# cartographer-project/cartographer

Hardware: AMD Instinct MI355X
Metric: candidate poses scored/sec (higher is better)
Workload: dtype u8/int32; 1 GPU; C2: 2D FastCorrelativeScanMatcher MatchFullSubmap (branch and bound): 1000-point scan vs 1 400x400 submap(s) per GPU, depth 7, full-angle search, m...; submaps_per_gpu=1, rotations=2373, found=1

## Files before the change

cartographer_amd/csrc/cmx_common.h:

```cpp
#ifndef CMX_COMMON_H_
#define CMX_COMMON_H_

#include <hip/hip_runtime.h>

#include <cstdarg>
#include <cstdint>
#include <cstdio>
#include <cstring>
#include <functional>
#include <mutex>
#include <string>
#include <vector>

#include "../../include/cartographer_mi355x.h"

namespace cmx {

void SetLastError(const char* fmt, ...);
const char* LastError();

struct HipError {
  cmx_status status;
};

// ... 30 lines not shown
    SetLastError("exception: %s", e.what());
    return CMX_DEVICE_ERROR;
  }
}

#define CMX_DEBUG_OPTIONS(X)                                                                      \
  X(rt2d_legacy)                 \
  X(rt2d_tile)                                        \
  X(rt2d_groups)                                   \
  X(rt2d_target)                                    \
  X(rt2d_lds_kb)                                         \
  X(rt2d_no_image_cache)             \
  X(rt2d_parts)                                 \
  X(rt2d_host_par)         \
  X(rt2d_tables_serial)    \
  X(rt2d_first_part)       \
  X(rt2d_image_kernels)    \
  X(rt2d_no_lane)          \
  X(rt2d_parts_pool)       \
  X(rt2d_grid_share)       \
  X(rt2d_unfused)            \
  X(rt2d_no_bounds)        \
  X(rt2d_bounds)           \
  X(rt2d_bounds_fused)     \
  X(rt2d_bounds_level)     \
  X(rt2d_bounds_verify)    \
  X(rt2d_tsdf_batch_legacy)  \
  X(rt2d_tsdf_batch_bulk)  \
  X(rt2d_tsdf_verify)      \
  X(timeline)                  \
  X(trace)                       \
  X(host_trace)                          \
  X(launch_serial)         \
  X(sync)                      \
  X(no_copy_kernels)             \
  X(timing)                \
  X(no_direct_results)     \
  X(frontier_capacity)     \
  X(comm_virtual_ranks)    \
  X(comm_force_rccl)       \
  X(fast2d_unfused)                    \
  X(fast2d_store_scans)                   \
  X(fast2d_fused_threads)                            \
  X(fast2d_fanout)         \
  X(fast2d_group)          \
  X(fast2d_group_verify)   \
  X(fast2d_levels_per_stage)                                    \
  X(fast2d_wave_levels)                        \
  X(fast2d_xcd_affinity)                          \
  X(fast2d_queue)          \
  X(fast2d_queue_blocks)                \
  X(fast2d_queue_capacity)              \
  X(fast2d_queue_lost)       \
  X(filters_generic)       \
  X(fast3d_byte_loads)                             \
  X(fast3d_affinity)                              \
  X(fast3d_no_families)                             \
  X(fast3d_no_oct)                                         \
  X(fast3d_batch)                                                 \
  X(fast3d_chunk_cells)    \
  X(rt3d_legacy)                  \
  X(rt3d_no_tiles)                      \
  X(rt3d_verify)                  \
  X(rt3d_no_rotblocks)              \
  X(rt3d_rotblock_permille)  \
  X(rt3d_crosscheck)           \
  X(rt3d_expand_all)       \
  X(rt3d_unstaged)                                     \
  X(rt3d_no_boxes)                            \
  X(rt3d_report)                                             \
  X(rt3d_segments)                         \
  X(rt3d_group_rotations)                                  \
  X(rt3d_group_tile_kb)                                   \
  X(rt3d_group_float)                          \
  X(rt3d_cand_threads)                                   \
  X(rt3d_cand_rotations)                                    \
  X(rt3d_cand_tile_kb)
struct DebugOptions {
#define CMX_DEBUG_FIELD(name) int name = 0;
  CMX_DEBUG_OPTIONS(CMX_DEBUG_FIELD)
#undef CMX_DEBUG_FIELD
};
const DebugOptions& Debug();
bool DebugSet(const char* name, int value);

void UseDevice(int device);

void ParallelFor(int n, int serial_below, const std::function<void(int)>& fn);

class LaunchTurn {
 public:
  LaunchTurn();
  ~LaunchTurn();
  LaunchTurn(const LaunchTurn&) = delete;
  LaunchTurn& operator=(const LaunchTurn&) = delete;
 private:
  bool held_;
};

class HostLane {
 public:
  HostLane();
  ~HostLane();
  HostLane(const HostLane&) = delete;
  HostLane& operator=(const HostLane&) = delete;
  void Run(std::function<void()> fn);
// ... 157 lines not shown
```

cartographer_amd/csrc/fast_2d.hip:

```cpp
#include <algorithm>
#include <chrono>
#include <cstring>
#include <memory>
#include <type_traits>
#include <utility>

#include "fast_2d_device.h"
#include "fast_2d_internal.h"

namespace cmx {
namespace {

constexpr int kSeedsPerProblem = 64;

constexpr int kMaxStages = kMaxDepth + 2;

constexpr int kCountStride = 32;
constexpr int kQueues = 2048;
struct alignas(8) QueueCtl {
  int head;
  int reserved;
  int pad[30];
};
struct Counters {
  int frontier[kMaxStages][kSubLists * kCountStride];
  int leaves[kSubLists * kCountStride];
  int frontier_overflow;
  int leaf_overflow;
  unsigned wave_gathers;
  int blocks_done;
  int pad[28];
  unsigned gathers_shard[16 * kCountStride];
  unsigned queue_stats[16 * kCountStride];
  QueueCtl queue[kQueues];
};

struct CountersSummary {
  int leaves[kSubLists];
  int frontier_total[kMaxStages];
  int frontier_overflow;
  int leaf_overflow;
  unsigned wave_gathers;
  int pad;
  unsigned queue_stats[8];
};

struct NodeList {
  Node2D* nodes;
  int* counts;
  int sub_capacity;
};

__device__ __forceinline__ int ListReserve(const NodeList& list, int sub, int m) {
  return atomicAdd(&list.counts[sub * kCountStride], m);
}
__device__ __forceinline__ bool ListStore(const NodeList& list, int sub, int slot,
                                          const Node2D& nd) {
  if (slot >= list.sub_capacity) return false;
  list.nodes[static_cast<size_t>(sub) * list.sub_capacity + slot] = nd;
  return true;
}
__device__ __forceinline__ int ListMaxCount(const NodeList& list) {
  const int lane = threadIdx.x & 63;
  return WaveMax(min(list.counts[lane * kCountStride], list.sub_capacity));
}

__device__ __forceinline__ int NodeProblem(const Node2D& nd) { return nd.problem & 0xffffff; }
__device__ __forceinline__ int NodeLevel(const Node2D& nd) { return nd.problem >> 24; }

__device__ __forceinline__ Node2D CoarseNode(const Fast2DProblem& P, int problem, int s,
                                             int local) {
  const int2 dims = P.coarse_dims[s];
  const int4 bd = P.bounds[s];
  const int step = 1 << (P.depth - 1);
  const int ix = local / dims.y, iy = local - ix * dims.y;
  const int c = s * P.coarse_stride + local;
  Node2D nd;
  nd.problem = problem | ((P.depth - 1) << 24);
  nd.scan = s;
  nd.dx = bd.x + ix * step;
  nd.dy = bd.z + iy * step;
  nd.score = P.coarse_score[c];
  nd.coarse_index = c;
  nd.path = 0;
  nd.coarse_score = nd.score;
  return nd;
}

struct SeedScratch {
  int hist[1024];
  int wave_total[4];
  int threshold_bin;
  int found_scan;
  int total;
};

__device__ __forceinline__ bool PickSeed(const Fast2DProblem& P, int n, int want,
                                         SeedScratch* sh, int* scan_out) {
  const int tid = threadIdx.x, lane = tid & 63, T = blockDim.x;
  for (int i = tid; i < 1024; i += T) sh->hist[i] = 0;
  if (tid == 0) { sh->found_scan = -1; sh->total = 0; }
  __syncthreads();
  const int S = P.num_scans;
  const long long range = 255ll * n + 1;
  const auto* scan_best = AsGlobal(P.scan_best);
  const auto* coarse_dims = AsGlobal(P.coarse_dims);
  const bool grouped = P.group > 1;
  const auto best_of = [&](int s) -> int {
    if (grouped) {
      const int first = s - s % kFusedGroup;
      if (s != first + (S - first >= kFusedGroup ? 1 : 0)) return -1;
    }
    return scan_best[s].x;
  };
  constexpr int kOwn = 16;
  int own[kOwn];
#pragma unroll
  for (int k = 0; k < kOwn; ++k) {
    const int s = tid + k * T;
    own[k] = s < S ? best_of(s) : -1;
  }
  int total = 0;
#pragma unroll
  for (int k = 0; k < kOwn; ++k)
    if (own[k] >= 0) atomicAdd(&sh->hist[static_cast<int>(own[k] * 1024ll / range)], 1);
  for (int s = tid + kOwn * T; s < S; s += T) {
    const int b = best_of(s);
    if (b >= 0) atomicAdd(&sh->hist[static_cast<int>(b * 1024ll / range)], 1);
  }
  if (want == 0) {
    for (int s = tid; s < S; s += T) total += coarse_dims[s].x * coarse_dims[s].y;
    total = WaveSum(total);
    if (lane == 0 && total) atomicAdd(&sh->total, total);
  }
  __syncthreads();
  if (tid < 64) {
    int mine = 0;
#pragma unroll
    for (int k = 0; k < 16; ++k) mine += sh->hist[1023 - 16 * lane - k];
// ... 168 lines not shown
  };
  if (quads_by_buffer) {
    if (cached) walk(std::true_type{}, std::true_type{});
    else walk(std::false_type{}, std::true_type{});
  } else {
    if (cached) walk(std::true_type{}, std::false_type{});
    else walk(std::false_type{}, std::false_type{});
  }
  s00 = WaveSum(s00); s01 = WaveSum(s01); s10 = WaveSum(s10); s11 = WaveSum(s11);
  const int wave = threadIdx.x >> 6;
  if ((threadIdx.x & 63) == 0) {
    sh->partial[wave][0] = s00; sh->partial[wave][1] = s01;
    sh->partial[wave][2] = s10; sh->partial[wave][3] = s11;
  }
  __syncthreads();
  if (threadIdx.x < 64) {
    const int k = threadIdx.x & 3;
    const bool valid = ((k >> 1) == 0 || vx) && ((k & 1) == 0 || vy);
    const int total = sh->partial[0][k] + sh->partial[1][k] + sh->partial[2][k] + sh->partial[3][k];
    const float mine = valid ? ToScoreCtx(ctx, total) : -1.f;
    int rank = 0, nvalid = 0;
#pragma unroll
    for (int j = 0; j < 4; ++j) {
      const float other = __shfl(mine, j, 64);
      if (other >= 0.f) ++nvalid;
      if (j != k && other >= 0.f && (other > mine || (other == mine && j < k))) ++rank;
    }
    if (threadIdx.x < 4) {
      sh->child_score[k] = mine;
      sh->rank[k] = rank;
      if (k == 0) sh->nvalid = nvalid;
    }
  }
  __syncthreads();
}

__device__ __forceinline__ Node2D MakeChild(const Node2D& nd, int k, int child_level,
                                            const ChildScratch& sh) {
  Node2D child = nd;
  child.problem = NodeProblem(nd) | (child_level << 24);
  child.dx = nd.dx + (k >> 1) * (1 << child_level);
  child.dy = nd.dy + (k & 1) * (1 << child_level);
  child.score = sh.child_score[k];
  child.path = nd.path | (static_cast<unsigned>(sh.rank[k]) << (2 * child_level));
  return child;
}

__device__ __forceinline__ void RecordLeaf(const Node2D& leaf, const NodeList& leaves,
                                           Counters* __restrict__ counters) {
  const int sub = blockIdx.x & (kSubLists - 1);
  if (!ListStore(leaves, sub, ListReserve(leaves, sub, 1), leaf)) counters->leaf_overflow = 1;
}

__global__ void __launch_bounds__(256, 4)
DiveKernel(const Fast2DProblem* __restrict__ problems, ProblemState* __restrict__ states, int n,
           NodeList leaves, Counters* __restrict__ counters) {
  const int problem = blockIdx.y;
  const Fast2DProblem& P = problems[problem];
  ProblemState& st = states[problem];
  if (st.error) return;
  __shared__ BlockContext ctx;
  __shared__ ChildScratch sh;
  __shared__ Node2D cur;
  __shared__ SeedScratch seed_scratch;
  const int per_seed = P.group > 1 ? kFusedGroup : 1;
  if (static_cast<int>(blockIdx.x) >= kSeedsPerProblem * per_seed) return;
  int seed_scan;
  const bool have_seed = PickSeed(P, n, blockIdx.x / per_seed, &seed_scratch, &seed_scan);
  if (blockIdx.x == 0 && threadIdx.x == 0) st.coarse_total = seed_scratch.total;
  if (!have_seed) return;
  if (per_seed > 1) {
    seed_scan = seed_scan - seed_scan % kFusedGroup + static_cast<int>(blockIdx.x) % per_seed;
    if (seed_scan >= P.num_scans) return;
  }
  const Node2D seed = CoarseNode(P, problem, seed_scan, P.scan_best[seed_scan].y);
  if (threadIdx.x == 0) cur = seed;
  LoadContext(P, n, seed.scan, &ctx);
  const int depth = NodeLevel(seed) + 1;
  unsigned long long scored = 0;
  for (int child_level = depth - 2; child_level >= 0; --child_level) {
    const Node2D nd = cur;
    ScoreChildren(ctx, nd.dx, nd.dy, child_level, &sh);
    scored += sh.nvalid;
    if (threadIdx.x == 0) {
      for (int k = 0; k < 4; ++k)
        if (sh.child_score[k] >= 0.f && sh.rank[k] == 0) cur = MakeChild(nd, k, child_level, sh);
    }
    __syncthreads();
  }
  if (threadIdx.x == 0) {
    const Node2D leaf = cur;
    if (leaf.score > ctx.min_score) {
      RecordLeaf(leaf, leaves, counters);
      atomicMax(&st.best_bits, __float_as_uint(leaf.score));
    }
    atomicAdd(&st.scored_shard[blockIdx.x & (kStatShards - 1)], scored);
    atomicAdd(&st.expanded_shard[blockIdx.x & (kStatShards - 1)],
              static_cast<unsigned long long>(depth - 1));
  }
}

__global__ void __launch_bounds__(256)
FilterCoarseKernel(const Fast2DProblem* __restrict__ problems,
                   const ProblemState* __restrict__ states, int n, int chunk, int num_chunks,
                   int strict, int affinity, NodeList out, Counters* __restrict__ counters) {
  const int problem = blockIdx.y;
  const Fast2DProblem& P = problems[problem];
  const int lane = threadIdx.x & 63;
  const int s = blockIdx.x * 4 + __builtin_amdgcn_readfirstlane(threadIdx.x >> 6);
  if (s >= P.num_scans || states[problem].error) return;
  if (s % num_chunks != chunk) return;
  const float best = __uint_as_float(states[problem].best_bits);
  const float top = ToScore(P, P.scan_best[s].x, n);
  if (strict ? !(top > best) : (top < best)) return;
  const int2 dims = P.coarse_dims[s];
  const int count = dims.x * dims.y;
  const int base = s * P.coarse_stride;
  const auto* scores = AsGlobal(P.coarse_score) + base;
  float ahead[4];
#pragma unroll
  for (int k = 0; k < 4; ++k) ahead[k] = k * kWave + lane < count ? scores[k * kWave + lane] : 0.f;
  for (int c0 = 0; c0 < count; c0 += kWave) {
    const int sub = affinity ? (problem & 7) + 8 * ((s + (c0 >> 6)) & 7)
                             : (s + blockIdx.y + (c0 >> 6)) & (kSubLists - 1);
    const int c = c0 + lane;
    bool keep = false;
    if (c < count) {
      float score;
      switch (c0 >> 6) {
        case 0: score = ahead[0]; break;
        case 1: score = ahead[1]; break;
        case 2: score = ahead[2]; break;
        case 3: score = ahead[3]; break;
        default: score = scores[c];
      }
      keep = strict ? (score > best) : (score >= best);
    }
    const unsigned long long mask = __ballot(keep);
    if (mask == 0) continue;
    int first = 0;
    if (lane == 0) first = ListReserve(out, sub, __popcll(mask));
    first = __builtin_amdgcn_readfirstlane(first);
    if (keep) {
      const int slot = first + __popcll(mask & ((1ull << lane) - 1));
      if (!ListStore(out, sub, slot, CoarseNode(P, problem, s, c))) counters->frontier_overflow = 1;
    }
  }
}

constexpr int kWaveStatProblems = 1024;

__global__ void __launch_bounds__(256)
// ... 584 lines not shown
__device__ __forceinline__ bool Steal(const TreeQueue& Q, Counters* __restrict__ counters,
                                      int home, int queues, unsigned salt, int windows,
                                      int max_lost, Node2D* out, unsigned* lost_races,
                                      unsigned* slot_rereads) {
  const int lane = threadIdx.x & 63;
  int lost = 0;
  for (int w = 0; w < windows; ++w) {
    const int base = static_cast<int>((static_cast<unsigned>(home) * 2654435761u + salt * 40503u + w * 64u) %
                                      static_cast<unsigned>(queues));
    const int mine = (base + lane) % queues;
    const unsigned long long hr =
        LoadAgent(reinterpret_cast<const unsigned long long*>(&counters->queue[mine].head));
    const int head = static_cast<int>(hr & 0xffffffffu);
    const int reserved = min(static_cast<int>(hr >> 32), Q.capacity);
    const unsigned long long avail = __ballot(reserved > head);
    if (avail == 0) continue;
    int skip = static_cast<int>((salt + home) % static_cast<unsigned>(__popcll(avail)));
    unsigned long long rest = avail;
    while (skip-- > 0) rest &= rest - 1;
    const int l = __ffsll(static_cast<long long>(rest)) - 1;
    const int q = (base + l) % queues;
    const int slot = __builtin_amdgcn_readlane(head, l);
    if (TakeSlot(counters, q, slot)) {
      ReadSlot(Q, q, slot, out, slot_rereads);
      return true;
    }
    ++*lost_races;
    if (++lost >= max_lost) return false;
    --w;
    ++salt;
  }
  return false;
}

constexpr int kChainCells = 16;
constexpr uint32_t kNoCell = 0x80008000u;

__device__ __forceinline__ void RecordLeafAgent(const Node2D& leaf, const NodeList& leaves,
                                                int sub, Counters* __restrict__ counters) {
  const int slot = ListReserve(leaves, sub, 1);
  if (slot >= leaves.sub_capacity) {
    __hip_atomic_store(&counters->leaf_overflow, 1, __ATOMIC_RELAXED, __HIP_MEMORY_SCOPE_AGENT);
    return;
  }
  unsigned long long v[4];
  __builtin_memcpy(v, &leaf, sizeof(Node2D));
  unsigned long long* at = reinterpret_cast<unsigned long long*>(
      &leaves.nodes[static_cast<size_t>(sub) * leaves.sub_capacity + slot]);
#pragma unroll
  for (int k = 0; k < 4; ++k)
    __hip_atomic_store(&at[k], v[k], __ATOMIC_RELAXED, __HIP_MEMORY_SCOPE_AGENT);
}

__global__ void __launch_bounds__(256)
TreeQueueKernel(const Fast2DProblem* __restrict__ problems, ProblemState* __restrict__ states, int n,
                NodeList in, TreeQueue Q, NodeList leaves, Counters* __restrict__ counters,
                SelectState* __restrict__ sel, BestLeaf* __restrict__ best_out, int num_problems,
                ProblemState* __restrict__ states_out, CountersSummary* __restrict__ summary,
                const unsigned* __restrict__ tail_dev, unsigned* __restrict__ tail_host,
                int tail_words, int counters_trace, int max_lost) {
  static_assert(sizeof(Node2D) == 32, "a node is eight words: eight granules, four leaf stores");
  const int lane = threadIdx.x & 63;
  const int wave_id = blockIdx.x * 4 + __builtin_amdgcn_readfirstlane(threadIdx.x >> 6);
  const int num_waves = gridDim.x * 4;
  const int queues = min(num_waves, kQueues);
  const int home = wave_id % queues;
  unsigned steals = 0;
  unsigned long long scored = 0, expanded = 0;
  unsigned gathers = 0;
  unsigned q_pops = 0, q_lost = 0, q_rereads = 0, q_pushed = 0, q_listed = 0, q_chains = 0;
  int stat_problem = -1;
  const auto flush_stats = [&]() {
    if (lane == 0 && stat_problem >= 0 && expanded) {
      ProblemState& st = states[stat_problem];
      atomicAdd(&st.scored_shard[wave_id & (kStatShards - 1)], scored);
      atomicAdd(&st.expanded_shard[wave_id & (kStatShards - 1)], expanded);
    }
    scored = expanded = 0;
  };
  const int in_slots = ListMaxCount(in) * kSubLists;
  int round = 0;
  Node2D mine{};
  unsigned mine_bits = 0;
  bool round_loaded = false, share_done = false;
  bool pushed_any = false;
  Node2D nd;
  for (;;) {
    bool have = false;
    while (!have && !share_done) {
      if (!round_loaded) {
        if (wave_id + static_cast<long long>(round) * 64 * num_waves >= in_slots) { share_done = true; break; }
        const long long i = wave_id + (static_cast<long long>(round) * 64 + lane) * num_waves;
        ++round;
        mine_bits = 0;
        if (i < in_slots) {
          const int in_sub = static_cast<int>(i & (kSubLists - 1)), j = static_cast<int>(i / kSubLists);
          if (j < min(in.counts[in_sub * kCountStride], in.sub_capacity)) {
            mine = in.nodes[static_cast<size_t>(in_sub) * in.sub_capacity + j];
            mine_bits = max(__float_as_uint(fmaxf(mine.score, 0.f)), 1u);
          }
        }
        round_loaded = true;
      }
      const unsigned top = static_cast<unsigned>(WaveMax(static_cast<int>(mine_bits)));
      const float bound_now = __uint_as_float(LoadAgent(&states[0].best_bits));
      if (top == 0 || (num_problems == 1 && __uint_as_float(top) < bound_now)) {
        round_loaded = false;
        continue;
      }
      const int l = __ffsll(static_cast<long long>(__ballot(mine_bits == top))) - 1;
      nd.problem = __builtin_amdgcn_readlane(mine.problem, l);
      nd.scan = __builtin_amdgcn_readlane(mine.scan, l);
      nd.dx = __builtin_amdgcn_readlane(mine.dx, l);
      nd.dy = __builtin_amdgcn_readlane(mine.dy, l);
      nd.score = __uint_as_float(__builtin_amdgcn_readlane(__float_as_uint(mine.score), l));
      nd.coarse_index = __builtin_amdgcn_readlane(mine.coarse_index, l);
      nd.path = __builtin_amdgcn_readlane(mine.path, l);
      nd.coarse_score =
          __uint_as_float(__builtin_amdgcn_readlane(__float_as_uint(mine.coarse_score), l));
      if (lane == l) mine_bits = 0;
      have = true;
      ++q_listed;
    }
    if (!have) {
      if (!(pushed_any && PopHome(Q, counters, home, &nd, &q_lost, &q_rereads)) &&
          !Steal(Q, counters, home, queues, ++steals, 2, max_lost, &nd, &q_lost, &q_rereads))
        break;
      ++q_pops;
    }
    const int problem = __builtin_amdgcn_readfirstlane(NodeProblem(nd));
    const Fast2DProblem& P = problems[problem];
    ProblemState& st = states[problem];
    float best = __uint_as_float(LoadAgent(&st.best_bits));
    if (nd.score < best) continue;
    if (problem != stat_problem) { flush_stats(); stat_problem = problem; }
    ++q_chains;
    const auto* pts = AsGlobal(P.discrete) + static_cast<size_t>(nd.scan) * n;
    uint32_t cell[kChainCells];
#pragma unroll
    for (int j = 0; j < kChainCells; ++j) {
      const int i = j * kWave + lane;
      cell[j] = kNoCell;
      if (j * kWave < n) cell[j] = i < n ? pts[i] : kNoCell;
    }
    const int4 bd = P.bounds[nd.scan];
    const float min_score = P.min_score;
    for (;;) {
      const int child_level = __builtin_amdgcn_readfirstlane(NodeLevel(nd) - 1);
      const LevelDesc& Lm = P.level[child_level];
      const int half = 1 << child_level;
      const int ndx = __builtin_amdgcn_readfirstlane(nd.dx), ndy = __builtin_amdgcn_readfirstlane(nd.dy);
      const bool vx = ndx + half <= bd.y, vy = ndy + half <= bd.w;
      const int ax = ndx + 2 * half - 1, ay = ndy + 2 * half - 1;
      const int parent_ub = SumUpperBound(P, nd.score, n);
      struct { int qx, qy, qtx; } L;
      L.qx = __builtin_amdgcn_readfirstlane(Lm.qx);
      L.qy = __builtin_amdgcn_readfirstlane(Lm.qy);
      L.qtx = __builtin_amdgcn_readfirstlane(Lm.qtx);
      const unsigned long long quads_address = reinterpret_cast<unsigned long long>(Lm.quads);
      const unsigned long long quads_uniform =
          static_cast<unsigned long long>(static_cast<unsigned>(
              __builtin_amdgcn_readfirstlane(static_cast<unsigned>(quads_address)))) |
          (static_cast<unsigned long long>(static_cast<unsigned>(
               __builtin_amdgcn_readfirstlane(static_cast<unsigned>(quads_address >> 32)))) << 32);
      const unsigned long long quad_bytes =
          static_cast<unsigned long long>((L.qy + 3) >> 2) * static_cast<unsigned>(L.qtx) * 128ull;
      const __amdgpu_buffer_rsrc_t quad_rsrc = __builtin_amdgcn_make_buffer_rsrc(
          reinterpret_cast<uint32_t*>(quads_uniform), 0, static_cast<int>(quad_bytes), 0x00020000);
      typedef unsigned short Halves __attribute__((ext_vector_type(2)));
      uint32_t even = 0, odd = 0;
      int seen_max = 0;
      bool dead = false;
      const auto gather = [&](auto first_tag, auto count_tag) {
// ... 269 lines not shown
                        std::chrono::steady_clock::now() - t0).count();
}

void SearchRun::PrepareStrictRetry() {
  CMX_REQUIRE(num_chunks < (1 << 12), "branch-and-bound overflow not resolvable");
  if (h_tail.summary->frontier_overflow) num_chunks *= 4;
  strict = 1;
  for (int p = 0; p < num; ++p) {
    const float floor_score = std::max(batch.h_problems[p].min_score, 0.f);
    unsigned floor_bits;
    std::memcpy(&floor_bits, &floor_score, sizeof(float));
    if (h_tail.states[p].best_bits > floor_bits) h_tail.states[p].best_bits -= 1;
  }
  CMX_HIP(hipMemcpyAsync(batch.d_states, h_tail.states, num * sizeof(ProblemState),
                         hipMemcpyHostToDevice, ws.stream));
  CMX_HIP(hipMemsetAsync(d_counters, 0, sizeof(Counters), ws.stream));
}

void RunDepthOne(SearchRun& run) {
  Workspace& ws = run.ws;
  SelectDepthOneKernel<<<run.num, 1024, 0, ws.stream>>>(
      run.batch.d_problems, run.batch.d_states, run.n, run.d_tail.best, run.d_tail.states);
  CMX_HIP(hipGetLastError());
  RecordEvent(ws.ev_end, ws.stream);
  run.FetchResults(false);
}

bool QueueSearchPossible(const SearchRun& run) {
  bool queue_ok = QueueSearchWanted(run.n, run.num);
  for (const Fast2DProblem& P : run.batch.h_problems) {
    queue_ok = queue_ok && (P.recompute_scans == 0 || P.store_scans != 0);
    for (int l = 0; l + 1 < run.depth; ++l)
      queue_ok = queue_ok && static_cast<unsigned long long>((P.level[l].qy + 3) >> 2) *
                                     static_cast<unsigned>(P.level[l].qtx) * 128ull < (1ull << 31);
  }
  return queue_ok;
}

enum class QueueOutcome { kDone, kLeafOverflow, kQueueOverflow };

QueueOutcome RunQueueSearch(SearchRun& run, std::unique_ptr<LaunchTurn> turn) {
  Workspace& ws = run.ws;
  const PreparedBatch& batch = run.batch;
  BatchResult* result = run.result;
  const int num = run.num, n = run.n;
  const long long wanted = std::max<long long>(1ll << 20, 65536ll * num);
  int sub_capacity = static_cast<int>(std::min<long long>(wanted, 1ll << 23) / kQueues);
  if (Debug().fast2d_queue_capacity > 0) sub_capacity = Debug().fast2d_queue_capacity;
  TreeQueue queue;
  queue.capacity = sub_capacity;
  queue.slots = static_cast<unsigned long long*>(ws.tagged[0].Acquire(
      static_cast<size_t>(kQueues) * sub_capacity * 8 * sizeof(unsigned long long), ws.stream,
      &queue.epoch));
  run.d_front[0] = ws.dev[10].ReserveAs<Node2D>(run.frontier_capacity);
  FilterCoarseKernel<<<dim3(DivUp(batch.max_scans, 4), num), 256, 0, ws.stream>>>(
      batch.d_problems, batch.d_states, n, 0, 1, 0, 0, run.Front(0),
      run.d_counters);
  run.Mark("filter");
  RecordEvent(ws.ev_x0, ws.stream);
  const int blocks = Debug().fast2d_queue_blocks > 0
                         ? Debug().fast2d_queue_blocks
                         : std::min(2048, 256 * std::max(1, (num + 3) / 4));
  TreeQueueKernel<<<blocks, 256, 0, ws.stream>>>(
      batch.d_problems, batch.d_states, n, run.Front(0), queue, run.leaf_list, run.d_counters,
      run.d_tail.sel, run.d_tail.best, num, run.d_tail.states, run.d_tail.summary,
      run.d_tail.words(), run.PublishTo(), run.h_tail.num_words(),
      batch.trace && batch.trace->enabled() ? 1 : 0,
      Debug().fast2d_queue_lost > 0 ? Debug().fast2d_queue_lost : 3);
  run.Mark("queue");
  CMX_HIP(hipGetLastError());
  RecordEvent(ws.ev_x1, ws.stream);
  result->expansion_launches = 1;
  RecordEvent(ws.ev_end, ws.stream);
  turn.reset();
  run.FetchResults(run.direct);
  const CountersSummary& h_counters = *run.h_tail.summary;
  result->expansion_lookups = 64ll * h_counters.wave_gathers;
  for (int p = 0; p < num; ++p)
    for (int k = 0; k < kStatShards; ++k)
      result->expansion_nodes += run.h_tail.states[p].expanded_shard[k];
  if (h_counters.leaf_overflow) return QueueOutcome::kLeafOverflow;
  if (h_counters.frontier_overflow) return QueueOutcome::kQueueOverflow;
  return QueueOutcome::kDone;
}

void RunLevelSynchronous(SearchRun& run) {
  Workspace& ws = run.ws;
  const PreparedBatch& batch = run.batch;
  BatchResult* result = run.result;
  const int num = run.num, n = run.n;
  const CountersSummary& h_counters = *run.h_tail.summary;
  const int kLevelsPerStage = std::max(0, Debug().fast2d_levels_per_stage);
  const int kWaveLevels = Debug().fast2d_wave_levels > 0 ? Debug().fast2d_wave_levels - 1 : -1;
  const int levels_per_stage = kLevelsPerStage > 0 ? kLevelsPerStage : (num < 4 ? kMaxDepth : 2);
  const int wave_levels = kWaveLevels >= 0 ? kWaveLevels : (num < 4 ? 1 : 2);
  const int affinity_override = Debug().fast2d_xcd_affinity;
  const int affinity = affinity_override ? affinity_override - 1 : (num >= 16 ? 1 : 0);
  const int wide_blocks = std::min(4096, 1024 * std::max(1, (num + 3) / 4));
  const int narrow_blocks = std::min(4096, 512 * std::max(1, (num + 3) / 4));
  run.d_front[0] = ws.dev[10].ReserveAs<Node2D>(run.frontier_capacity);
  run.d_front[1] = ws.dev[11].ReserveAs<Node2D>(run.frontier_capacity);
  for (;;) {
    const int strict = run.strict;
    for (int chunk = 0; chunk < run.num_chunks; ++chunk) {
      if (chunk > 0 || strict)
        CMX_HIP(hipMemsetAsync(run.d_counters->frontier, 0, sizeof(run.d_counters->frontier),
                               ws.stream));
      FilterCoarseKernel<<<dim3(DivUp(batch.max_scans, 4), num), 256, 0, ws.stream>>>(
          batch.d_problems, batch.d_states, n, chunk, run.num_chunks, strict, affinity,
          run.Front(0), run.d_counters);
      run.Mark("filter");
      int stage = 0;
      int top = run.depth - 1;
      const bool timed = !strict && chunk == 0 && num >= 4;
      if (timed) RecordEvent(ws.ev_x0, ws.stream);
      for (int used = 0; used < wave_levels && top - 1 >= 1; ++used, --top, ++stage) {
        ExpandWaveKernel<<<used == 0 ? wide_blocks : narrow_blocks, 256, 0, ws.stream>>>(
            batch.d_problems, batch.d_states, n, run.Front(stage), strict, affinity,
// ... 17 lines not shown
        run.d_counters, run.d_tail.summary, run.d_tail.words(), run.PublishTo(),
        run.h_tail.num_words());
    run.Mark("select");
    CMX_HIP(hipGetLastError());
    RecordEvent(ws.ev_end, ws.stream);
    run.FetchResults(run.direct);
    if (!strict) {
      for (int st = 0; st < result->expansion_launches; ++st)
        result->expansion_nodes += h_counters.frontier_total[st];
      result->expansion_lookups = 64ll * h_counters.wave_gathers;
    }
    if (!h_counters.frontier_overflow && !h_counters.leaf_overflow) break;
    run.PrepareStrictRetry();
  }
}

void TraceListSizes(const CountersSummary& h_counters) {
  fprintf(stderr, "[cmx trace] list sizes:");
  for (int st = 0; st < kMaxStages; ++st)
    if (h_counters.frontier_total[st])
      fprintf(stderr, " frontier[%d]=%d", st, h_counters.frontier_total[st]);
  long long leaves = 0;
  for (int k = 0; k < kSubLists; ++k) leaves += h_counters.leaves[k];
  fprintf(stderr, " leaves=%lld\n", leaves);
  const unsigned* q = h_counters.queue_stats;
  if (q[5])
    fprintf(stderr, "[cmx trace] work queue: %u chains (%u nodes from the list, %u popped), %u "
            "pushed, %u lost races, %u slot re-reads\n", q[5], q[4], q[0], q[3], q[1], q[2]);
}

}

bool QueueSearchWanted(int n, int num) {
  return Debug().fast2d_queue != 2 && n <= kChainCells * kWave && (num < 4 || Debug().fast2d_queue == 1);
}

void ReserveSearchScratch(Workspace& ws, int num, PreparedBatch* batch) {
  batch->d_misc = static_cast<char*>(ws.dev[14].Reserve(SearchMiscBytes(num)));
  batch->num_counter_words = static_cast<int>(sizeof(Counters) / sizeof(int));
}

thread_local long long g_host_wait_ns = 0;

void RunBranchAndBound(Workspace& ws, const PreparedBatch& batch, BatchResult* result) {
  const int num = batch.num_problems;
  const int depth = batch.h_problems[0].depth;
  for (const Fast2DProblem& P : batch.h_problems)
    CMX_REQUIRE(P.depth == depth, "all matchers of a batch must share branch_and_bound_depth");
  SearchRun run(ws, batch, result);
  if (depth == 1) {
    RunDepthOne(run);
  } else {
    std::unique_ptr<LaunchTurn> turn(new LaunchTurn);
    DiveKernel<<<dim3(kSeedsPerProblem * (batch.any_group ? kFusedGroup : 1), num), 256, 0, ws.stream>>>(
        batch.d_problems, batch.d_states, run.n, run.leaf_list, run.d_counters);
    run.Mark("seed+dive");
    bool searched = false;
    if (QueueSearchPossible(run)) {
      switch (RunQueueSearch(run, std::move(turn))) {
        case QueueOutcome::kDone:
          searched = true;
          break;
        case QueueOutcome::kLeafOverflow:
          run.PrepareStrictRetry();
          break;
        case QueueOutcome::kQueueOverflow:
          CMX_HIP(hipMemsetAsync(run.d_counters, 0, sizeof(Counters), ws.stream));
          break;
      }
    }
    turn.reset();
    if (!searched) RunLevelSynchronous(run);
  }

  result->best.assign(run.h_tail.best, run.h_tail.best + num);
  result->states.assign(run.h_tail.states, run.h_tail.states + num);
  if (depth > 1) {
    if (batch.trace && batch.trace->enabled()) TraceListSizes(*run.h_tail.summary);
    result->d_leaves = run.leaf_list.nodes;
    result->leaf_sub_capacity = run.leaf_list.sub_capacity;
    result->leaf_counts.assign(run.h_tail.summary->leaves, run.h_tail.summary->leaves + kSubLists);
  }
  result->device_ms = ElapsedMs(ws.ev_begin, ws.ev_end);
  result->dominant_ms = ElapsedMs(ws.ev_k0, ws.ev_k1);
  if (result->expansion_launches > 0) result->expansion_ms = ElapsedMs(ws.ev_x0, ws.ev_x1);
}

}
```

cartographer_amd/csrc/fast_2d_coarse.hip:

```cpp
#include <algorithm>
#include <cmath>
#include <cstring>
#include <memory>
#include <mutex>
#include <vector>

#include "fast_2d_device.h"
#include "fast_2d_internal.h"

namespace cmx {
namespace {

constexpr int kMaxBuckets = 4096;
constexpr int kMaxCoarsePerScan = 4096;
constexpr int kMaxAccCells = 12288;

__global__ void __launch_bounds__(256)
PrepScansKernel(const Fast2DProblem* __restrict__ problems, const float* __restrict__ xyz, int n,
                ProblemState* __restrict__ states, int* __restrict__ counters_words,
                int num_counter_words) {
  if (counters_words)
    for (int i = (blockIdx.y * gridDim.x + blockIdx.x) * blockDim.x + threadIdx.x;
         i < num_counter_words; i += gridDim.x * gridDim.y * blockDim.x)
      counters_words[i] = 0;
// ... 952 lines not shown
    out->initial[p] = init;
    int r = -1;
    for (size_t k = 0; k < rotations.size(); ++k)
      if (rotations[k].step == h.step && rotations[k].num_angular == h.num_angular) r = static_cast<int>(k);
    if (r < 0) {
      r = static_cast<int>(rotations.size());
      rotations.push_back(Rotation{h.step, h.num_angular, HostRotationTable(h.step, h.num_angular),
                                   rotation_floats});
      rotation_floats += 2 * static_cast<size_t>(h.num_scans);
    }
    rotation_of[p] = r;
    discrete_total += static_cast<size_t>(h.num_scans) * n;
    scans_total += h.num_scans + 1;
    const long long cap = Q.ax * Q.ay * h.num_scans;
    Fast2DProblem& P = out->h_problems[p];
    P.coarse_capacity = static_cast<int>(cap);
    P.coarse_stride = static_cast<int>(Q.ax * Q.ay);
    P.use_planes = Q.use_planes;
    P.use_fused = Q.use_fused;
    P.write_all_discrete = out->write_all_discrete ? 1 : 0;
    P.group = Q.group;
    P.group_verify = Debug().fast2d_group_verify;
    P.timeline = nullptr;
    coarse_total += cap;
  }

  uint32_t* d_discrete =
      ws.dev[2].ReserveAs<uint32_t>(discrete_total + (any_unfused ? 2 * discrete_total + 2 : 0));
  uint2* d_sorted = reinterpret_cast<uint2*>(d_discrete + discrete_total + (discrete_total & 1));
  int4* d_bounds = ws.dev[3].ReserveAs<int4>(scans_total);
  int2* d_dims = ws.dev[4].ReserveAs<int2>(2 * scans_total);
  int2* d_scan_best = d_dims + scans_total;
  int* d_sorted_count = ws.dev[5].ReserveAs<int>(scans_total);
  float* d_cscore = ws.dev[6].ReserveAs<float>(coarse_total);
  int* d_csum = ws.dev[7].ReserveAs<int>(coarse_total);
  const size_t problems_bytes = (num * sizeof(Fast2DProblem) + 255) & ~size_t(255);
  const size_t states_bytes = (num * sizeof(ProblemState) + 255) & ~size_t(255);
  const size_t upload_bytes = problems_bytes + states_bytes + rotation_floats * sizeof(float);
  char* d_upload = static_cast<char*>(ws.dev[8].Reserve(upload_bytes));
  out->d_problems = reinterpret_cast<Fast2DProblem*>(d_upload);
  out->d_states = reinterpret_cast<ProblemState*>(d_upload + problems_bytes);
  const float* d_rotations = reinterpret_cast<const float*>(d_upload + problems_bytes + states_bytes);
  char* h_upload = static_cast<char*>(ws.pinned[1].Reserve(upload_bytes));
  Fast2DProblem* h_prob = reinterpret_cast<Fast2DProblem*>(h_upload);
  ProblemState* h_state = reinterpret_cast<ProblemState*>(h_upload + problems_bytes);
  float* h_rotations = reinterpret_cast<float*>(h_upload + problems_bytes + states_bytes);
  for (const Rotation& r : rotations)
    std::memcpy(h_rotations + r.offset, r.table->data(), r.table->size() * sizeof(float2));

  if (TimelineEnabled() && any_fused) {
    int max_scans = 0;
    for (const HostSearch& h : out->search) max_scans = std::max(max_scans, h.num_scans);
    out->timeline_blocks = (max_scans + 255) / 256 * 256 * num;
    const size_t bytes = static_cast<size_t>(out->timeline_blocks) * kTimelineStamps * 8;
    out->d_timeline = static_cast<unsigned long long*>(ws.dev[15].Reserve(bytes));
    CMX_HIP(hipMemsetAsync(out->d_timeline, 0, bytes, ws.stream));
  }
  const int store_override = Debug().fast2d_store_scans;
  const int store_scans =
      store_override ? store_override - 1 : ((num >= 4 || QueueSearchWanted(n, num)) ? 1 : 0);
  size_t disc_off = 0, scan_off = 0, coarse_off = 0;
  for (int p = 0; p < num; ++p) {
    const Fast2DMatcher& m = *matchers[p];
    const cmx_grid2d_limits& lim = m.limits();
    const HostSearch& h = out->search[p];
    Fast2DProblem& P = out->h_problems[p];
    P.timeline = out->d_timeline;
    P.xyz = d_xyz;
    P.recompute_scans = (P.use_fused && !P.write_all_discrete) ? 1 : 0;
    P.store_scans = store_scans;
    for (int i = 0; i < m.depth(); ++i) P.level[i] = m.level(i);
    P.depth = m.depth();
    P.nx = lim.num_x_cells; P.ny = lim.num_y_cells;
    P.nl = h.nl;
    P.res = lim.resolution; P.max_x = lim.max_x; P.max_y = lim.max_y;
    P.tx = static_cast<float>(out->initial[p].x);
    P.ty = static_cast<float>(out->initial[p].y);
    {
      const float ha = 0.5f * static_cast<float>(out->initial[p].theta);
      P.init_qw = std::cos(ha);
      P.init_qz = std::sin(ha) * 1.f;
    }
    P.num_scans = h.num_scans;
    P.inv_res = 1.0 / P.res;
    P.scan_rot = reinterpret_cast<const float2*>(d_rotations + rotations[rotation_of[p]].offset);
    P.min_s = m.min_s();
    P.score_scale = m.score_scale();
    P.min_score = min_of(p);
    P.planes = m.planes();
    P.planes_group = m.planes_group();
    P.plane_i = m.plane_i();
    P.plane_j = m.plane_j();
    P.plane_stride = m.plane_stride();
    P.discrete = d_discrete + disc_off;
    P.sorted = d_sorted + disc_off;
    P.bounds = d_bounds + scan_off;
    P.coarse_dims = d_dims + scan_off;
    P.scan_best = d_scan_best + scan_off;
    P.sorted_count = d_sorted_count + scan_off;
    P.coarse_score = d_cscore + coarse_off;
    P.coarse_sum = d_csum + coarse_off;
    h_prob[p] = P;
    std::memset(&h_state[p], 0, sizeof(ProblemState));
    const float bound = std::max(min_of(p), 0.f);
    std::memcpy(&h_state[p].best_bits, &bound, sizeof(float));
    disc_off += static_cast<size_t>(h.num_scans) * n;
    scan_off += h.num_scans + 1;
// ... 100 lines not shown
```

cartographer_amd/csrc/fast_2d_internal.h:

```cpp
#ifndef CMX_FAST_2D_INTERNAL_H_
#define CMX_FAST_2D_INTERNAL_H_

#include <vector>

#include "scan_matching_2d.h"

namespace cmx {

constexpr int kGroupDilation = 2;
constexpr int kFusedGroup = 3;
constexpr int kSubLists = 64;

struct HostSearch {
  int num_angular;
  double step;
  int num_scans;
  int nl;
};

struct PreparedBatch {
  StageTrace* trace = nullptr;
  int num_problems = 0;
  int n = 0;
  int max_scans = 0;
  long long plane_acc_cells = 0;
  std::vector<HostSearch> search;
  std::vector<cmx_pose2d> initial;
  Fast2DProblem* d_problems = nullptr;
  ProblemState* d_states = nullptr;
  std::vector<Fast2DProblem> h_problems;
  char* d_misc = nullptr;
  int num_counter_words = 0;
  bool write_all_discrete = false;
  unsigned long long* d_timeline = nullptr;
  int timeline_blocks = 0;
  bool any_group = false;
  size_t fused_lds = 0;
  int fused_acc = 0, fused_threads = 0;
  const float* d_xyz = nullptr;
};

struct BatchResult {
  std::vector<BestLeaf> best;
  std::vector<ProblemState> states;
  double device_ms = 0., dominant_ms = 0.;
  double expansion_ms = 0.;
  int expansion_launches = 0;
  long long expansion_nodes = 0, expansion_lookups = 0;
  const Node2D* d_leaves = nullptr;
  int leaf_sub_capacity = 0;
  std::vector<int> leaf_counts;
};

struct PlanMatcher {
  cmx_grid2d_limits limits;
  double linear_search_window, angular_search_window;
  int depth;
  bool planes, planes_group;
  int plane_i, plane_j, plane_stride;
};
PlanMatcher PlanMatcherOf(const Fast2DMatcher& m);
PlanMatcher PlanMatcherOf(const cmx_fast2d_options& options, const cmx_grid2d_limits& limits);

// ... 35 lines not shown
```

cartographer_amd/csrc/fast_2d_match.hip:

```cpp
#include <algorithm>
#include <atomic>
#include <chrono>
#include <cmath>
#include <cstring>
#include <functional>
#include <vector>

#include "../../include/cartographer_mi355x_debug.h"
#include "fast_2d_internal.h"

namespace cmx {
namespace {

float MaxRangeXY(const float* xyz, int n) {
  float m = 0.f;
  for (int i = 0; i < n; ++i) {
    const float x = xyz[3 * i], y = xyz[3 * i + 1];
    m = std::max(m, std::sqrt(x * x + y * y));
  }
  return m;
}

struct ScoreIndex {
  float score;
// ... 173 lines not shown
      total.device_ms += st.device_ms;
      total.dominant_kernel_ms += st.dominant_kernel_ms;
      total.expansion_ms += st.expansion_ms;
      total.expansion_launches += st.expansion_launches;
      total.expansion_nodes += st.expansion_nodes;
      total.expansion_lookups += st.expansion_lookups;
    }
    if (stats) *stats = total;
    return;
  }
  const auto t_call = std::chrono::steady_clock::now();
  g_host_wait_ns = 0;
  WorkspaceLease ws(device);
  const float* d_xyz;
  float max_range;
  if (cloud) {
    CMX_REQUIRE(cloud->device == device, "cloud and matcher are on different devices");
    d_xyz = cloud->xyz;
    max_range = cloud->max_range_xy;
  } else {
    CMX_REQUIRE(host_xyz != nullptr, "point cloud is null");
    float* buf = ws->dev[0].ReserveAs<float>(3 * static_cast<size_t>(n));
    CMX_HIP(hipMemcpyAsync(buf, host_xyz, 3 * sizeof(float) * n, hipMemcpyHostToDevice,
                           ws->stream));
    d_xyz = buf;
    max_range = MaxRangeXY(host_xyz, n);
  }
  RecordEvent(ws->ev_begin, ws->stream);
  PreparedBatch batch;
  StageTrace trace(ws->stream);
  batch.trace = &trace;
  ReserveSearchScratch(*ws, num, &batch);
  PrepareAndScoreCoarse(*ws, matchers.data(), num, initial, full_submap, d_xyz, n, max_range,
                        min_score, &batch, full_flags, min_scores);
  BatchResult result;
  RunBranchAndBound(*ws, batch, &result);
  if (matchers[0]->depth() > 1) {
    ResolveTies(*ws, batch, &result);
  } else {
    ResolveDepthOne(batch, &result.best, result.states);
  }
  if (Debug().host_trace) {
    g_host_total_ns += std::chrono::duration_cast<std::chrono::nanoseconds>(
                           std::chrono::steady_clock::now() - t_call).count();
    g_host_waited_ns += g_host_wait_ns;
    const long long calls = ++g_host_calls;
    if (calls % 2000 == 0)
      fprintf(stderr, "[cmx host] fast2d: %lld calls, mean %.1f us per call, of which %.1f us in the final synchronisation\n",
              calls, g_host_total_ns.load() * 1e-3 / calls, g_host_waited_ns.load() * 1e-3 / calls);
  }
  trace.Report();
  if (batch.d_timeline)
    ReportTimeline("PrepScoreFusedKernel", batch.d_timeline, batch.timeline_blocks, ws->stream);
  if (trace.enabled()) {
    for (int p = 0; p < std::min(num, 4); ++p) {
      unsigned long long ex = 0;
      for (int k = 0; k < kStatShards; ++k) ex += result.states[p].expanded_shard[k];
      fprintf(stderr, "[cmx trace] problem %d: coarse %d expanded %llu found %d ties %d\n", p,
              result.states[p].coarse_total, ex, result.best[p].found, result.best[p].ties);
    }
  }
  CheckProblemErrors(result);
  cmx_match_stats total{};
  for (int p = 0; p < num; ++p) {
    const BestLeaf& b = result.best[p];
    const HostSearch& h = batch.search[p];
    const bool ok = b.found && b.score > (min_scores ? min_scores[p] : min_score);
    found[p] = ok ? 1 : 0;
    if (ok) {
      const double res = matchers[p]->limits().resolution;
      const double cx = -b.dy * res, cy = -b.dx * res;
      const double orientation = (b.scan - h.num_angular) * h.step;
      scores[p] = b.score;
      poses[p].x = batch.initial[p].x + cx;
      poses[p].y = batch.initial[p].y + cy;
      poses[p].theta = batch.initial[p].theta + orientation;
    }
    total.candidates_scored += result.states[p].coarse_total;
    total.coarse_candidates += result.states[p].coarse_total;
    for (int k = 0; k < kStatShards; ++k) {
      total.candidates_scored += result.states[p].scored_shard[k];
      total.nodes_expanded += result.states[p].expanded_shard[k];
    }
    total.num_scans += h.num_scans;
  }
  total.device_ms = result.device_ms;
  total.dominant_kernel_ms = result.dominant_ms;
  total.expansion_ms = result.expansion_ms;
  total.expansion_launches = result.expansion_launches;
  total.expansion_nodes = result.expansion_nodes;
  total.expansion_lookups = result.expansion_lookups;
  if (stats) *stats = total;
}

}
}

using cmx::Guard;

extern "C" {

cmx_status cmx_fast2d_match(const cmx_fast2d* matcher, const cmx_pose2d* initial_pose_estimate,
                            const float* point_cloud_xyz, int32_t num_points, float min_score,
                            int32_t* found, float* score, cmx_pose2d* pose_estimate,
                            cmx_match_stats* stats) {
  return Guard([&] {
// ... 218 lines not shown
```

Baseline: 10.19 billion candidates/s.

## Feed tree queue directly from coarse scores, skipping the filter kernel

```diff
diff --git a/cartographer_amd/csrc/cmx_common.h b/cartographer_amd/csrc/cmx_common.h
--- a/cartographer_amd/csrc/cmx_common.h
+++ b/cartographer_amd/csrc/cmx_common.h
@@ -106,6 +106,7 @@
   X(fast2d_queue_blocks)                \
   X(fast2d_queue_capacity)              \
   X(fast2d_queue_lost)       \
+  X(fast2d_queue_intake)   \
   X(filters_generic)       \
   X(fast3d_byte_loads)                             \
   X(fast3d_affinity)                              \
diff --git a/cartographer_amd/csrc/fast_2d.hip b/cartographer_amd/csrc/fast_2d.hip
--- a/cartographer_amd/csrc/fast_2d.hip
+++ b/cartographer_amd/csrc/fast_2d.hip
@@ -10,8 +10,6 @@
 
 namespace cmx {
 namespace {
-
-constexpr int kSeedsPerProblem = 64;
 
 constexpr int kMaxStages = kMaxDepth + 2;
 
@@ -68,23 +66,29 @@
 __device__ __forceinline__ int NodeProblem(const Node2D& nd) { return nd.problem & 0xffffff; }
 __device__ __forceinline__ int NodeLevel(const Node2D& nd) { return nd.problem >> 24; }
 
-__device__ __forceinline__ Node2D CoarseNode(const Fast2DProblem& P, int problem, int s,
-                                             int local) {
-  const int2 dims = P.coarse_dims[s];
-  const int4 bd = P.bounds[s];
+__device__ __forceinline__ Node2D CoarseNodeAt(const Fast2DProblem& P, int problem, int s,
+                                               int local, int min_x, int min_y, int dims_y,
+                                               float score) {
   const int step = 1 << (P.depth - 1);
-  const int ix = local / dims.y, iy = local - ix * dims.y;
+  const int ix = local / dims_y, iy = local - ix * dims_y;
   const int c = s * P.coarse_stride + local;
   Node2D nd;
   nd.problem = problem | ((P.depth - 1) << 24);
   nd.scan = s;
-  nd.dx = bd.x + ix * step;
-  nd.dy = bd.z + iy * step;
-  nd.score = P.coarse_score[c];
+  nd.dx = min_x + ix * step;
+  nd.dy = min_y + iy * step;
+  nd.score = score;
   nd.coarse_index = c;
   nd.path = 0;
-  nd.coarse_score = nd.score;
+  nd.coarse_score = score;
   return nd;
+}
+
+__device__ __forceinline__ Node2D CoarseNode(const Fast2DProblem& P, int problem, int s,
+                                             int local) {
+  const int4 bd = P.bounds[s];
+  return CoarseNodeAt(P, problem, s, local, bd.x, bd.z, P.coarse_dims[s].y,
+                      P.coarse_score[s * P.coarse_stride + local]);
 }
 
 struct SeedScratch {
@@ -359,10 +363,15 @@
   if (!ListStore(leaves, sub, ListReserve(leaves, sub, 1), leaf)) counters->leaf_overflow = 1;
 }
 
+template <bool kTimeline>
 __global__ void __launch_bounds__(256, 4)
 DiveKernel(const Fast2DProblem* __restrict__ problems, ProblemState* __restrict__ states, int n,
-           NodeList leaves, Counters* __restrict__ counters) {
+           NodeList leaves, Counters* __restrict__ counters, unsigned long long* timeline) {
   const int problem = blockIdx.y;
+  const auto stamp = [&](int k) {
+    if constexpr (kTimeline) Stamp(timeline, blockIdx.y * gridDim.x + blockIdx.x, k);
+  };
+  stamp(0);
   const Fast2DProblem& P = problems[problem];
   ProblemState& st = states[problem];
   if (st.error) return;
@@ -375,6 +384,7 @@
   int seed_scan;
   const bool have_seed = PickSeed(P, n, blockIdx.x / per_seed, &seed_scratch, &seed_scan);
   if (blockIdx.x == 0 && threadIdx.x == 0) st.coarse_total = seed_scratch.total;
+  stamp(1);
   if (!have_seed) return;
   if (per_seed > 1) {
     seed_scan = seed_scan - seed_scan % kFusedGroup + static_cast<int>(blockIdx.x) % per_seed;
@@ -383,6 +393,7 @@
   const Node2D seed = CoarseNode(P, problem, seed_scan, P.scan_best[seed_scan].y);
   if (threadIdx.x == 0) cur = seed;
   LoadContext(P, n, seed.scan, &ctx);
+  stamp(2);
   const int depth = NodeLevel(seed) + 1;
   unsigned long long scored = 0;
   for (int child_level = depth - 2; child_level >= 0; --child_level) {
@@ -405,6 +416,7 @@
     atomicAdd(&st.expanded_shard[blockIdx.x & (kStatShards - 1)],
               static_cast<unsigned long long>(depth - 1));
   }
+  stamp(3);
 }
 
 __global__ void __launch_bounds__(256)
@@ -1095,10 +1107,12 @@
     __hip_atomic_store(&at[k], v[k], __ATOMIC_RELAXED, __HIP_MEMORY_SCOPE_AGENT);
 }
 
+template <bool kListIntake>
 __global__ void __launch_bounds__(256)
 TreeQueueKernel(const Fast2DProblem* __restrict__ problems, ProblemState* __restrict__ states, int n,
-                NodeList in, TreeQueue Q, NodeList leaves, Counters* __restrict__ counters,
-                SelectState* __restrict__ sel, BestLeaf* __restrict__ best_out, int num_problems,
+                NodeList in, int max_scans, TreeQueue Q, NodeList leaves,
+                Counters* __restrict__ counters, SelectState* __restrict__ sel,
+                BestLeaf* __restrict__ best_out, int num_problems,
                 ProblemState* __restrict__ states_out, CountersSummary* __restrict__ summary,
                 const unsigned* __restrict__ tail_dev, unsigned* __restrict__ tail_host,
                 int tail_words, int counters_trace, int max_lost) {
@@ -1121,47 +1135,109 @@
     }
     scored = expanded = 0;
   };
-  const int in_slots = ListMaxCount(in) * kSubLists;
+  const int in_slots = kListIntake ? ListMaxCount(in) * kSubLists : 0;
   int round = 0;
   Node2D mine{};
   unsigned mine_bits = 0;
+  unsigned held[4] = {0, 0, 0, 0};
+  int pair = wave_id;
+  const int num_pairs = max_scans * num_problems;
+  int cur_problem = 0, cur_scan = 0, cur_count = 0, cur_min_x = 0, cur_min_y = 0, cur_dims_y = 1;
+  int round_first = 0, next_first = 0;
   bool round_loaded = false, share_done = false;
   bool pushed_any = false;
   Node2D nd;
   for (;;) {
     bool have = false;
     while (!have && !share_done) {
-      if (!round_loaded) {
-        if (wave_id + static_cast<long long>(round) * 64 * num_waves >= in_slots) { share_done = true; break; }
-        const long long i = wave_id + (static_cast<long long>(round) * 64 + lane) * num_waves;
-        ++round;
-        mine_bits = 0;
-        if (i < in_slots) {
-          const int in_sub = static_cast<int>(i & (kSubLists - 1)), j = static_cast<int>(i / kSubLists);
-          if (j < min(in.counts[in_sub * kCountStride], in.sub_capacity)) {
-            mine = in.nodes[static_cast<size_t>(in_sub) * in.sub_capacity + j];
-            mine_bits = max(__float_as_uint(fmaxf(mine.score, 0.f)), 1u);
+      if constexpr (kListIntake) {
+        if (!round_loaded) {
+          if (wave_id + static_cast<long long>(round) * 64 * num_waves >= in_slots) { share_done = true; break; }
+          const long long i = wave_id + (static_cast<long long>(round) * 64 + lane) * num_waves;
+          ++round;
+          mine_bits = 0;
+          if (i < in_slots) {
+            const int in_sub = static_cast<int>(i & (kSubLists - 1)), j = static_cast<int>(i / kSubLists);
+            if (j < min(in.counts[in_sub * kCountStride], in.sub_capacity)) {
+              mine = in.nodes[static_cast<size_t>(in_sub) * in.sub_capacity + j];
+              mine_bits = max(__float_as_uint(fmaxf(mine.score, 0.f)), 1u);
+            }
           }
+          round_loaded = true;
         }
-        round_loaded = true;
-      }
-      const unsigned top = static_cast<unsigned>(WaveMax(static_cast<int>(mine_bits)));
-      const float bound_now = __uint_as_float(LoadAgent(&states[0].best_bits));
-      if (top == 0 || (num_problems == 1 && __uint_as_float(top) < bound_now)) {
-        round_loaded = false;
-        continue;
-      }
-      const int l = __ffsll(static_cast<long long>(__ballot(mine_bits == top))) - 1;
-      nd.problem = __builtin_amdgcn_readlane(mine.problem, l);
-      nd.scan = __builtin_amdgcn_readlane(mine.scan, l);
-      nd.dx = __builtin_amdgcn_readlane(mine.dx, l);
-      nd.dy = __builtin_amdgcn_readlane(mine.dy, l);
-      nd.score = __uint_as_float(__builtin_amdgcn_readlane(__float_as_uint(mine.score), l));
-      nd.coarse_index = __builtin_amdgcn_readlane(mine.coarse_index, l);
-      nd.path = __builtin_amdgcn_readlane(mine.path, l);
-      nd.coarse_score =
-          __uint_as_float(__builtin_amdgcn_readlane(__float_as_uint(mine.coarse_score), l));
-      if (lane == l) mine_bits = 0;
+        const unsigned top = static_cast<unsigned>(WaveMax(static_cast<int>(mine_bits)));
+        const float bound_now = __uint_as_float(LoadAgent(&states[0].best_bits));
+        if (top == 0 || (num_problems == 1 && __uint_as_float(top) < bound_now)) {
+          round_loaded = false;
+          continue;
+        }
+        const int l = __ffsll(static_cast<long long>(__ballot(mine_bits == top))) - 1;
+        nd.problem = __builtin_amdgcn_readlane(mine.problem, l);
+        nd.scan = __builtin_amdgcn_readlane(mine.scan, l);
+        nd.dx = __builtin_amdgcn_readlane(mine.dx, l);
+        nd.dy = __builtin_amdgcn_readlane(mine.dy, l);
+        nd.score = __uint_as_float(__builtin_amdgcn_readlane(__float_as_uint(mine.score), l));
+        nd.coarse_index = __builtin_amdgcn_readlane(mine.coarse_index, l);
+        nd.path = __builtin_amdgcn_readlane(mine.path, l);
+        nd.coarse_score =
+            __uint_as_float(__builtin_amdgcn_readlane(__float_as_uint(mine.coarse_score), l));
+        if (lane == l) mine_bits = 0;
+      } else {
+        if (!round_loaded) {
+          if (next_first >= cur_count) {
+            if (pair >= num_pairs) { share_done = true; break; }
+            const int p = pair / max_scans, s = pair - p * max_scans;
+            pair += num_waves;
+            cur_count = next_first = 0;
+            const Fast2DProblem& PP = problems[p];
+            if (s >= PP.num_scans || states[p].error) continue;
+            const float bound = __uint_as_float(LoadAgent(&states[p].best_bits));
+            if (ToScore(PP, PP.scan_best[s].x, n) < bound) continue;
+            const int2 dims = PP.coarse_dims[s];
+            const int4 bd = PP.bounds[s];
+            cur_problem = p;
+            cur_scan = s;
+            cur_count = __builtin_amdgcn_readfirstlane(dims.x * dims.y);
+            cur_dims_y = __builtin_amdgcn_readfirstlane(dims.y);
+            cur_min_x = __builtin_amdgcn_readfirstlane(bd.x);
+            cur_min_y = __builtin_amdgcn_readfirstlane(bd.z);
+            if (cur_count <= 0) continue;
+          }
+          const Fast2DProblem& PP = problems[cur_problem];
+          const float bound = __uint_as_float(LoadAgent(&states[cur_problem].best_bits));
+          const auto* scores = AsGlobal(PP.coarse_score) + static_cast<size_t>(cur_scan) * PP.coarse_stride;
+          round_first = next_first;
+          next_first += 4 * kWave;
+          float score[4];
+#pragma unroll
+          for (int k = 0; k < 4; ++k) {
+            const int c = round_first + k * kWave + lane;
+            score[k] = c < cur_count ? scores[c] : -1.f;
+          }
+#pragma unroll
+          for (int k = 0; k < 4; ++k)
+            held[k] = score[k] < bound ? 0u : max(__float_as_uint(fmaxf(score[k], 0.f)), 1u);
+          round_loaded = true;
+        }
+        const unsigned top = static_cast<unsigned>(
+            WaveMax(static_cast<int>(max(max(held[0], held[1]), max(held[2], held[3])))));
+        const float bound_now = __uint_as_float(LoadAgent(&states[cur_problem].best_bits));
+        if (top == 0 || __uint_as_float(top) < bound_now) {
+          round_loaded = false;
+          continue;
+        }
+        const int mine_k = held[0] == top ? 0 : (held[1] == top ? 1 : (held[2] == top ? 2 : (held[3] == top ? 3 : -1)));
+        const int l = __ffsll(static_cast<long long>(__ballot(mine_k >= 0))) - 1;
+        const int k = __builtin_amdgcn_readlane(mine_k, l);
+#pragma unroll
+        for (int j = 0; j < 4; ++j)
+          if (lane == l && j == k) held[j] = 0;
+        const Fast2DProblem& PP = problems[cur_problem];
+        const int local = round_first + k * kWave + l;
+        const float score = top > 1u ? __uint_as_float(top)
+                                     : PP.coarse_score[static_cast<size_t>(cur_scan) * PP.coarse_stride + local];
+        nd = CoarseNodeAt(PP, cur_problem, cur_scan, local, cur_min_x, cur_min_y, cur_dims_y, score);
+      }
       have = true;
       ++q_listed;
     }
@@ -1537,18 +1613,21 @@
   queue.slots = static_cast<unsigned long long*>(ws.tagged[0].Acquire(
       static_cast<size_t>(kQueues) * sub_capacity * 8 * sizeof(unsigned long long), ws.stream,
       &queue.epoch));
-  run.d_front[0] = ws.dev[10].ReserveAs<Node2D>(run.frontier_capacity);
-  FilterCoarseKernel<<<dim3(DivUp(batch.max_scans, 4), num), 256, 0, ws.stream>>>(
-      batch.d_problems, batch.d_states, n, 0, 1, 0, 0, run.Front(0),
-      run.d_counters);
-  run.Mark("filter");
+  const bool list_intake = Debug().fast2d_queue_intake == 1;
+  if (list_intake) {
+    run.d_front[0] = ws.dev[10].ReserveAs<Node2D>(run.frontier_capacity);
+    FilterCoarseKernel<<<dim3(DivUp(batch.max_scans, 4), num), 256, 0, ws.stream>>>(
+        batch.d_problems, batch.d_states, n, 0, 1, 0, 0, run.Front(0),
+        run.d_counters);
+    run.Mark("filter");
+  }
   RecordEvent(ws.ev_x0, ws.stream);
   const int blocks = Debug().fast2d_queue_blocks > 0
                          ? Debug().fast2d_queue_blocks
                          : std::min(2048, 256 * std::max(1, (num + 3) / 4));
-  TreeQueueKernel<<<blocks, 256, 0, ws.stream>>>(
-      batch.d_problems, batch.d_states, n, run.Front(0), queue, run.leaf_list, run.d_counters,
-      run.d_tail.sel, run.d_tail.best, num, run.d_tail.states, run.d_tail.summary,
+  (list_intake ? TreeQueueKernel<true> : TreeQueueKernel<false>)<<<blocks, 256, 0, ws.stream>>>(
+      batch.d_problems, batch.d_states, n, run.Front(0), batch.max_scans, queue, run.leaf_list,
+      run.d_counters, run.d_tail.sel, run.d_tail.best, num, run.d_tail.states, run.d_tail.summary,
       run.d_tail.words(), run.PublishTo(), run.h_tail.num_words(),
       batch.trace && batch.trace->enabled() ? 1 : 0,
       Debug().fast2d_queue_lost > 0 ? Debug().fast2d_queue_lost : 3);
@@ -1672,8 +1751,12 @@
     RunDepthOne(run);
   } else {
     std::unique_ptr<LaunchTurn> turn(new LaunchTurn);
-    DiveKernel<<<dim3(kSeedsPerProblem * (batch.any_group ? kFusedGroup : 1), num), 256, 0, ws.stream>>>(
-        batch.d_problems, batch.d_states, run.n, run.leaf_list, run.d_counters);
+    unsigned long long* const dive_timeline =
+        batch.d_timeline ? batch.d_timeline + static_cast<size_t>(batch.timeline_blocks) * kTimelineStamps
+                         : nullptr;
+    (dive_timeline ? DiveKernel<true> : DiveKernel<false>)
+        <<<dim3(kSeedsPerProblem * (batch.any_group ? kFusedGroup : 1), num), 256, 0, ws.stream>>>(
+            batch.d_problems, batch.d_states, run.n, run.leaf_list, run.d_counters, dive_timeline);
     run.Mark("seed+dive");
     bool searched = false;
     if (QueueSearchPossible(run)) {
diff --git a/cartographer_amd/csrc/fast_2d_coarse.hip b/cartographer_amd/csrc/fast_2d_coarse.hip
--- a/cartographer_amd/csrc/fast_2d_coarse.hip
+++ b/cartographer_amd/csrc/fast_2d_coarse.hip
@@ -1028,7 +1028,8 @@
     int max_scans = 0;
     for (const HostSearch& h : out->search) max_scans = std::max(max_scans, h.num_scans);
     out->timeline_blocks = (max_scans + 255) / 256 * 256 * num;
-    const size_t bytes = static_cast<size_t>(out->timeline_blocks) * kTimelineStamps * 8;
+    const size_t bytes = (static_cast<size_t>(out->timeline_blocks) + kDiveTimelineBlocks * num) *
+                         kTimelineStamps * 8;
     out->d_timeline = static_cast<unsigned long long*>(ws.dev[15].Reserve(bytes));
     CMX_HIP(hipMemsetAsync(out->d_timeline, 0, bytes, ws.stream));
   }
diff --git a/cartographer_amd/csrc/fast_2d_internal.h b/cartographer_amd/csrc/fast_2d_internal.h
--- a/cartographer_amd/csrc/fast_2d_internal.h
+++ b/cartographer_amd/csrc/fast_2d_internal.h
@@ -9,6 +9,8 @@
 
 constexpr int kGroupDilation = 2;
 constexpr int kFusedGroup = 3;
+constexpr int kSeedsPerProblem = 64;
+constexpr int kDiveTimelineBlocks = kSeedsPerProblem * kFusedGroup;
 constexpr int kSubLists = 64;
 
 struct HostSearch {
diff --git a/cartographer_amd/csrc/fast_2d_match.hip b/cartographer_amd/csrc/fast_2d_match.hip
--- a/cartographer_amd/csrc/fast_2d_match.hip
+++ b/cartographer_amd/csrc/fast_2d_match.hip
@@ -249,6 +249,10 @@
   trace.Report();
   if (batch.d_timeline)
     ReportTimeline("PrepScoreFusedKernel", batch.d_timeline, batch.timeline_blocks, ws->stream);
+  if (batch.d_timeline && batch.h_problems[0].depth > 1)
+    ReportTimeline("DiveKernel",
+                   batch.d_timeline + static_cast<size_t>(batch.timeline_blocks) * kTimelineStamps,
+                   kDiveTimelineBlocks * num, ws->stream);
   if (trace.enabled()) {
     for (int p = 0; p < std::min(num, 4); ++p) {
       unsigned long long ex = 0;
```

Result: slower. 9.581 billion candidates/s (-6.0%).
